# wisamreid/HcUnet

Measured on AMD Instinct MI355X. Metric: training voxels/sec (fwd+bwd+step), 5-level 3D U-Net, 256×256×16×4 tiles, higher is better.
Workload: dtype fp32; 1 GPU; config 2: 3D U-Net feature_sizes=[8,16,32,64,128] fp32 train step (fwd + pixel BCE + bwd + Adam), B=2 per GPU, 256x256x16x4 volumes; global_batch=2, per_gpu_batch=2, input_dtype=fp32, parallelism=dp1

## Files before the change

### hcunet_amd/csrc/common.h

```cpp
#pragma once
#include <hip/hip_runtime.h>
#include <hip/hip_ext.h>
#include <cstddef>
#include <cstdint>
#include <algorithm>
#include <cstdlib>
#include <string>

typedef float floatx4 __attribute__((ext_vector_type(4)));
typedef short shortx8 __attribute__((ext_vector_type(8)));
typedef short shortx4 __attribute__((ext_vector_type(4)));
typedef short shortx2 __attribute__((ext_vector_type(2)));
typedef float floatx2 __attribute__((ext_vector_type(2)));
typedef unsigned int u32x2 __attribute__((ext_vector_type(2)));
typedef unsigned int u32x4 __attribute__((ext_vector_type(4)));
typedef __bf16 bf16x2 __attribute__((ext_vector_type(2)));

namespace hcu {

struct ChainRec {
  hipStream_t s = nullptr;
  hipEvent_t ev = nullptr;
  unsigned long n = 0;
};
// ... 311 lines not shown
  f.Cout = Cout;
  f.Cin_g = Cin_g;
  f.groups = groups;
  f.fold_mod = fold_mod;
  f.part_c = part_c;
  f.part_cs = part_cs;
  f.ACs = ACs;
  return f;
}
inline PwWgArgs pw_wgrad_args(const WGradFinalize &f, const void *A, const void *G, long nvox,
                              int ACs, int GCs) {
  PwWgArgs g{};
  g.A = static_cast<const uint16_t *>(A);
  g.G = static_cast<const uint16_t *>(G);
  g.partial = const_cast<float *>(f.partial);
  g.nvox = nvox;
  g.per_block = (nvox + f.KB - 1) / f.KB;
  g.ACs = ACs;
  g.GCs = GCs;
  g.ACR = f.ACs;
  g.GCR = f.Ntot;
  g.Mtot = f.Mtot;
  g.Ntot = f.Ntot;
  g.bias_row = f.Mtot > f.T * f.ACs ? 1 : 0;
  return g;
}
int launch_wgrad_finalize(const WGradFinalize &f, hipStream_t s);
constexpr int kWgfBatch = 24;
int launch_wgrad_finalize_batch(const WGradFinalize *fs, int n, hipStream_t s);


int launch_bn_fwd_finalize(const float *stats, int R, int statsW, int C, int Cs,
                           double count, const float *gamma, const float *beta,
                           float *run_mean, float *run_var, int64_t *nbt,
                           float eps, float momentum, int training, BNCoef coef,
                           hipStream_t s);
int launch_bn_bwd_finalize(const float *part, int R, int C, int Cs, int W, double count,
                           BNCoef coef, float *dgamma, float *dbeta, int training,
                           int accumulate, hipStream_t s);

int launch_maxpool_fwd(const float *y, const float *scale, const float *shift,
                       float *p, int B, int X, int Y, int Z, int Cs,
                       int kx, int ky, int kz, hipStream_t s, int bf = 0);

int bwd_rows(int64_t nvox, int Cs);
int launch_bn_bwd_reduce_dense(float *dA, const float *y, BNCoef coef,
                               int64_t nvox, int Cs, float *part, int R,
                               hipStream_t s, int bf = 0);
int pool_bwd_rows(int B, int X, int Y, int Z, int Cs, int kx, int ky, int kz);
int launch_bn_bwd_reduce_pool(const float *dP, const float *y, BNCoef coef,
                              float *dz, int B, int X, int Y, int Z, int Cs,
                              int kx, int ky, int kz, float *part, int R,
                              hipStream_t s, int bf = 0);
int launch_bn_bwd_apply(float *dz, const float *y, BNCoef coef, int64_t nvox,
                        int Cs, hipStream_t s, int bf = 0);

int launch_outconv_fwd(const float *y, BNCoef coef, const float *w,
                       const float *bias, float *pred, int B, int64_t V, int C,
                       int Cs, int Co, hipStream_t s, int bf = 0);
int outconv_bwd_rows(int64_t nvox, int Cs);
int launch_outconv_bwd(const float *dpred, const float *y, BNCoef coef,
                       const float *w, float *dz, int B, int64_t V, int C,
                       int Cs, int Co, float *part_bn, float *part_oc, int R,
                       hipStream_t s, int bf = 0);

int chansum_rows(int64_t nvox, int Cs);
int launch_chansum(const float *x, int64_t nvox, int Cs, float *part, int R,
                   hipStream_t s, int bf = 0);
int launch_reduce_partials(const float *part, int R, int W, int n, float *out,
                           int accumulate, hipStream_t s);

int launch_to_cl(const float *x, float *xcl, int B, int C, int Cs, int64_t V,
                 hipStream_t s, int bf = 0, int x_dtype = 0);
int launch_from_cl(const float *xcl, float *x, int B, int C, int Cs, int64_t V,
                   hipStream_t s, int bf = 0);

struct WPack {
  int on, CK, S, ICs, CoutW;
};
inline WPack wpack_of(const GConvArgs &a) {
  WPack p{};
  if (a.use_bconv && a.bes == 4) {
    const int T = a.KX * a.KY * a.KZ, TPS = 16 / a.CK;
    p.on = 1;
    p.CK = a.CK;
    p.S = (T + TPS - 1) / TPS;
    p.ICs = a.ICs;
    p.CoutW = a.CoutW;
    return p;
  }
  if (a.use_bconv) {
    const int T = a.KX * a.KY * a.KZ, TPS = 32 / a.CK;
    p.on = 3;
    p.CK = a.CK;
    p.S = (T + TPS - 1) / TPS;
    p.ICs = a.ICs;
    p.CoutW = a.CoutW;
    return p;
  }
  if (a.use_conv8) {
    p.on = 2;
    p.CK = a.ICs / 4;
    p.S = a.KX * a.KY * a.KZ;
    p.ICs = a.ICs;
    p.CoutW = 8;
    return p;
// ... 105 lines not shown
```

### hcunet_amd/csrc/pointwise.hip

```cpp
#include "common.h"
#include "timing.h"
#include <algorithm>

namespace hcu {

__device__ __forceinline__ float bnrelu(float y, float sc, float sh) {
  return fmaxf(fmaf(y, sc, sh), 0.f);
}
__device__ __forceinline__ float4 ld4(const float *p) {
  return *reinterpret_cast<const float4 *>(p);
}
__device__ __forceinline__ void st4(float *p, float4 v) {
  *reinterpret_cast<float4 *>(p) = v;
}
struct bf16_t {
  uint16_t v;
};
__device__ __forceinline__ float4 ld4(const bf16_t *p) {
  const uint2 u = *reinterpret_cast<const uint2 *>(p);
  return make_float4(bf_lo(u.x), bf_hi(u.x), bf_lo(u.y), bf_hi(u.y));
}
__device__ __forceinline__ void st4(bf16_t *p, float4 v) {
  *reinterpret_cast<uint2 *>(p) = make_uint2(pack_bf2(v.x, v.y), pack_bf2(v.z, v.w));
}
// ... 309 lines not shown
}

int launch_maxpool_fwd(const float *y, const float *scale, const float *shift,
                       float *p, int B, int X, int Y, int Z, int Cs, int kx, int ky,
                       int kz, hipStream_t s, int bf) {
  const int PX = X / kx, PY = Y / ky, PZ = Z / kz;
  const int64_t n = (int64_t)B * PX * PY * PZ * (Cs / 4);
  if (n >= (int64_t)1 << 31) return fail(4, "max_pool3d: more than 2^31 channel quads per launch");
  if (kx == 2 && ky == 2 && kz == 1 && n > 0) {
    const int N = bf ? 8 : 4;
    if (Cs % N == 0) {
      const int64_t nv = (int64_t)B * PX * PY * PZ * (Cs / N);
      HCU_TIMED(s, "maxpool221_kernel", 0.0, (double)(bf ? 2 : 4) * Cs * ((double)B * X * Y * Z + (double)B * PX * PY * PZ),
                HCU_BF_DISPATCH(bf, maxpool221_kernel, dim3((unsigned)((nv + 255) / 256)), dim3(256), 0, s,
                                (const T *)y, scale, shift, (T *)p, X, Y, Z, Cs, PX, PY, (uint32_t)nv,
                                pool_div(Cs * 4 / N, PX, PY, PZ)));
      HCU_CHECK_LAUNCH();
      return 0;
    }
  }
  HCU_TIMED(s, "maxpool_fwd_kernel", 0.0, 0.0,
            HCU_BF_DISPATCH(bf, maxpool_fwd_kernel, dim3(grid_for(n)), dim3(256), 0, s,
                            (const T *)y, scale, shift, (T *)p, B, X, Y, Z, Cs, kx, ky, kz, PX,
                            PY, PZ, pool_div(Cs, PX, PY, PZ)));
  HCU_CHECK_LAUNCH();
  return 0;
}

struct RedGeom {
  int tb;
  int64_t chunk;
  int64_t total;
};
__host__ __device__ inline RedGeom red_geom(int64_t nvox, int Cs, int R) {
  RedGeom g;
  const int C4 = Cs / 4;
  g.tb = C4 <= 256 ? (256 / C4) * C4 : C4;
  g.total = nvox * C4;
  int64_t per = (g.total + R - 1) / R;
  g.chunk = (per + g.tb - 1) / g.tb * g.tb;
  return g;
}
int bwd_rows(int64_t nvox, int Cs) {
  const int C4 = Cs / 4;
  const int tb = C4 <= 256 ? (256 / C4) * C4 : C4;
  const int64_t total = nvox * C4;
  int64_t r = (total + (int64_t)tb * 4 - 1) / ((int64_t)tb * 4);
  return (int)std::max<int64_t>(1, std::min<int64_t>(r, 1024));
}
int chansum_rows(int64_t nvox, int Cs) { return bwd_rows(nvox, Cs); }
int outconv_bwd_rows(int64_t nvox, int Cs) { return bwd_rows(nvox, Cs); }

template <int NV>
__device__ void block_reduce_c4(float (&v)[NV], float *lds, int tb, int C4,
                                float *out_row ) {
  const int tid = threadIdx.x;
  if (tid < tb)
    for (int k = 0; k < NV; ++k) lds[tid * NV + k] = v[k];
  __syncthreads();
  if (tid < C4) {
    float acc[NV];
    for (int k = 0; k < NV; ++k) acc[k] = 0.f;
    for (int t = tid; t < tb; t += C4)
      for (int k = 0; k < NV; ++k) acc[k] += lds[t * NV + k];
    for (int k = 0; k < NV; ++k) out_row[tid * NV + k] = acc[k];
  }
}

template <typename T>
__global__ void __launch_bounds__(256)
bn_bwd_reduce_dense_kernel(T *dA, const T *y, BNCoef coef, int64_t nvox,
                           int Cs, float *part, RedGeom g) {
  extern __shared__ __attribute__((aligned(16))) float lds[];
  const int C4 = Cs / 4, tid = threadIdx.x;
  float v[8] = {0, 0, 0, 0, 0, 0, 0, 0};
  if (tid < g.tb) {
    const int64_t beg = (int64_t)blockIdx.x * g.chunk;
    const int64_t end = std::min(beg + g.chunk, g.total);
    const int c = (int)((beg + tid) % C4) * 4;
    const float4 sc = ld4(coef.scale + c), sh = ld4(coef.shift + c);
    const float4 mu = ld4(coef.mean + c), is = ld4(coef.invstd + c);
    for (int64_t e = beg + tid; e < end; e += g.tb) {
      const size_t off = (size_t)e * 4;
      const float4 yy = ld4(y + off);
      float4 d = ld4(dA + off);
      d.x = fmaf(yy.x, sc.x, sh.x) > 0.f ? d.x : 0.f;
      d.y = fmaf(yy.y, sc.y, sh.y) > 0.f ? d.y : 0.f;
      d.z = fmaf(yy.z, sc.z, sh.z) > 0.f ? d.z : 0.f;
      d.w = fmaf(yy.w, sc.w, sh.w) > 0.f ? d.w : 0.f;
      st4(dA + off, d);
      v[0] += d.x;
      v[1] = fmaf(d.x, (yy.x - mu.x) * is.x, v[1]);
      v[2] += d.y;
      v[3] = fmaf(d.y, (yy.y - mu.y) * is.y, v[3]);
      v[4] += d.z;
      v[5] = fmaf(d.z, (yy.z - mu.z) * is.z, v[5]);
      v[6] += d.w;
      v[7] = fmaf(d.w, (yy.w - mu.w) * is.w, v[7]);
    }
  }
  block_reduce_c4<8>(v, lds, g.tb, C4, part + (size_t)blockIdx.x * Cs * 2);
}

int launch_bn_bwd_reduce_dense(float *dA, const float *y, BNCoef coef, int64_t nvox,
                               int Cs, float *part, int R, hipStream_t s, int bf) {
  const RedGeom g = red_geom(nvox, Cs, R);
  HCU_TIMED(s, "bn_bwd_reduce_dense_kernel", 0.0, 2.0 * nvox * Cs * (bf ? 2 : 4),
            HCU_BF_DISPATCH(bf, bn_bwd_reduce_dense_kernel, dim3(R), dim3(256),
                            (size_t)std::max(g.tb, 256) * 8 * 4, s, (T *)dA, (const T *)y, coef,
                            nvox, Cs, part, g));
  HCU_CHECK_LAUNCH();
  return 0;
}

template <typename T>
__global__ void __launch_bounds__(256)
bn_bwd_reduce_pool_kernel(const T *dP, const T *y, BNCoef coef, T *dz,
                          int B, int X, int Y, int Z, int Cs, int kx, int ky, int kz,
                          float *part, RedGeom g, PoolDiv dv) {
// ... 19 lines not shown
      float4 m = make_float4(-INFINITY, -INFINITY, -INFINITY, -INFINITY);
      int4 am = make_int4(-1, -1, -1, -1);
      int idx = 0;
      for (int i = 0; i < kx; ++i)
        for (int j = 0; j < ky; ++j)
          for (int k = 0; k < kz; ++k, ++idx) {
            const float4 t = ld4(y + ((((size_t)b * X + x0 + i) * Y + y0 + j) * Z + z0 + k) * Cs + c);
            const float a0 = bnrelu(t.x, sc.x, sh.x), a1 = bnrelu(t.y, sc.y, sh.y);
            const float a2 = bnrelu(t.z, sc.z, sh.z), a3 = bnrelu(t.w, sc.w, sh.w);
            if (a0 > m.x) { m.x = a0; am.x = idx; }
            if (a1 > m.y) { m.y = a1; am.y = idx; }
            if (a2 > m.z) { m.z = a2; am.z = idx; }
            if (a3 > m.w) { m.w = a3; am.w = idx; }
          }
      const float4 gp = ld4(dP + ((((size_t)b * PX + wx) * PY + wy) * PZ + wz) * Cs + c);
      for (int x = x0; x < x1; ++x)
        for (int yy = y0; yy < y1; ++yy)
          for (int z = z0; z < z1; ++z) {
            const size_t off = ((((size_t)b * X + x) * Y + yy) * Z + z) * Cs + c;
            float4 d = make_float4(0.f, 0.f, 0.f, 0.f);
            const bool inwin = x < x0 + kx && yy < y0 + ky && z < z0 + kz;
            if (inwin) {
              const int own = ((x - x0) * ky + (yy - y0)) * kz + (z - z0);
              const float4 yv = ld4(y + off);
              const float4 zv = make_float4(fmaf(yv.x, sc.x, sh.x), fmaf(yv.y, sc.y, sh.y),
                                            fmaf(yv.z, sc.z, sh.z), fmaf(yv.w, sc.w, sh.w));
              d.x = (am.x == own && zv.x > 0.f) ? gp.x : 0.f;
              d.y = (am.y == own && zv.y > 0.f) ? gp.y : 0.f;
              d.z = (am.z == own && zv.z > 0.f) ? gp.z : 0.f;
              d.w = (am.w == own && zv.w > 0.f) ? gp.w : 0.f;
              v[0] += d.x;
              v[1] = fmaf(d.x, (yv.x - mu.x) * is.x, v[1]);
              v[2] += d.y;
              v[3] = fmaf(d.y, (yv.y - mu.y) * is.y, v[3]);
              v[4] += d.z;
              v[5] = fmaf(d.z, (yv.z - mu.z) * is.z, v[5]);
              v[6] += d.w;
              v[7] = fmaf(d.w, (yv.w - mu.w) * is.w, v[7]);
            }
            st4(dz + off, d);
          }
    }
  }
  block_reduce_c4<8>(v, lds, g.tb, C4, part + (size_t)blockIdx.x * Cs * 2);
}

template <int N>
struct Win221 {
  float a[4][N], gp[N];
  int wx, wy, wz, b;
  bool ok;
};
template <typename T>
__global__ void __launch_bounds__(256)
bn_bwd_reduce_pool221_kernel(const T *dP, const T *y, BNCoef coef, T *dz, int X, int Y, int Z,
                             int Cs, float *part, RedGeom g, PoolDiv dv) {
  constexpr int N = VN<T>::N;
  extern __shared__ __attribute__((aligned(16))) float lds[];
  const int G = Cs / N, tid = threadIdx.x;
  const int PX = X / 2, PY = Y / 2;
  const size_t sy = (size_t)Z * Cs, sx = (size_t)Y * sy;
  float v[2 * N];
#pragma unroll
  for (int k = 0; k < 2 * N; ++k) v[k] = 0.f;
  if (tid < g.tb) {
    const int64_t beg = (int64_t)blockIdx.x * g.chunk;
    const int64_t end = std::min(beg + g.chunk, g.total);
    const int c = (int)((beg + tid) % G) * N;
    float sc[N], sh[N], mu[N], is[N];
    ldc<N>(coef.scale + c, sc);
    ldc<N>(coef.shift + c, sh);
    ldc<N>(coef.mean + c, mu);
    ldc<N>(coef.invstd + c, is);
    auto load = [&](int64_t e, Win221<N> &w) {
      w.ok = e < end;
      if (!w.ok) return;
      int q, gg;
      dv.c4.divmod((uint32_t)e, q, gg);
      dv.pz.divmod((uint32_t)q, q, w.wz);
      dv.py.divmod((uint32_t)q, q, w.wy);
      dv.px.divmod((uint32_t)q, w.b, w.wx);
      const size_t base = (((size_t)w.b * X + 2 * w.wx) * Y + 2 * w.wy) * sy + (size_t)w.wz * Cs + c;
      ldv(y + base, w.a[0]);
      ldv(y + base + sy, w.a[1]);
      ldv(y + base + sx, w.a[2]);
      ldv(y + base + sx + sy, w.a[3]);
      ldv(dP + ((((size_t)w.b * PX + w.wx) * PY + w.wy) * Z + w.wz) * Cs + c, w.gp);
    };
    auto finish = [&](const Win221<N> &w) {
      if (!w.ok) return;
      float d[4][N];
#pragma unroll
      for (int j = 0; j < N; ++j) {
        float m = -INFINITY;
        int am = -1;
        float zz[4];
#pragma unroll
        for (int t = 0; t < 4; ++t) {
          zz[t] = fmaf(w.a[t][j], sc[j], sh[j]);
          const float q = fmaxf(zz[t], 0.f);
          if (q > m) { m = q; am = t; }
        }
#pragma unroll
        for (int t = 0; t < 4; ++t) d[t][j] = (am == t && zz[t] > 0.f) ? w.gp[j] : 0.f;
      }
      const size_t base = (((size_t)w.b * X + 2 * w.wx) * Y + 2 * w.wy) * sy + (size_t)w.wz * Cs + c;
      stv(dz + base, d[0]);
      stv(dz + base + sy, d[1]);
      stv(dz + base + sx, d[2]);
      stv(dz + base + sx + sy, d[3]);
#pragma unroll
      for (int t = 0; t < 4; ++t)
#pragma unroll
        for (int j = 0; j < N; ++j) {
          v[2 * j] += d[t][j];
          v[2 * j + 1] = fmaf(d[t][j], (w.a[t][j] - mu[j]) * is[j], v[2 * j + 1]);
        }
      const bool lx = w.wx == PX - 1 && X > 2 * PX, ly = w.wy == PY - 1 && Y > 2 * PY;
      if (lx || ly) {
        float zero[N];
#pragma unroll
        for (int j = 0; j < N; ++j) zero[j] = 0.f;
        const int x1 = lx ? X : 2 * w.wx + 2, y1 = ly ? Y : 2 * w.wy + 2;
        for (int x = 2 * w.wx; x < x1; ++x)
          for (int yy = 2 * w.wy; yy < y1; ++yy)
            if (x >= 2 * w.wx + 2 || yy >= 2 * w.wy + 2)
              stv(dz + (((size_t)w.b * X + x) * Y + yy) * sy + (size_t)w.wz * Cs + c, zero);
      }
    };
    for (int64_t e = beg + tid; e < end; e += 2 * (int64_t)g.tb) {
      Win221<N> w0, w1;
      load(e, w0);
      load(e + g.tb, w1);
      finish(w0);
      finish(w1);
    }
  }
  if (tid < g.tb)
#pragma unroll
    for (int k = 0; k < 2 * N; ++k) lds[tid * 2 * N + k] = v[k];
  __syncthreads();
  if (tid < G) {
    float acc[2 * N];
#pragma unroll
    for (int k = 0; k < 2 * N; ++k) acc[k] = 0.f;
    for (int t = tid; t < g.tb; t += G)
#pragma unroll
      for (int k = 0; k < 2 * N; ++k) acc[k] += lds[t * 2 * N + k];
    float *out = part + (size_t)blockIdx.x * Cs * 2 + (size_t)tid * 2 * N;
#pragma unroll
    for (int k = 0; k < 2 * N; ++k) out[k] = acc[k];
  }
}

int pool_bwd_rows(int B, int X, int Y, int Z, int Cs, int kx, int ky, int kz) {
  return bwd_rows((int64_t)B * (X / kx) * (Y / ky) * (Z / kz), Cs);
}

int launch_bn_bwd_reduce_pool(const float *dP, const float *y, BNCoef coef, float *dz,
                              int B, int X, int Y, int Z, int Cs, int kx, int ky,
                              int kz, float *part, int R, hipStream_t s, int bf) {
  const RedGeom g = red_geom((int64_t)B * (X / kx) * (Y / ky) * (Z / kz), Cs, R);
  if (g.total >= (int64_t)1 << 31) return fail(4, "max_pool3d backward: more than 2^31 channel quads");
  const int N = bf ? 8 : 4;
  if (kx == 2 && ky == 2 && kz == 1 && Cs % N == 0) {
    const RedGeom gv = red_geom((int64_t)B * (X / 2) * (Y / 2) * Z, Cs * 4 / N, R);
    HCU_TIMED(s, "bn_bwd_reduce_pool221_kernel", 0.0,
              (double)(bf ? 2 : 4) * Cs * ((double)B * (X / 2) * (Y / 2) * Z + 2.0 * B * X * Y * Z),
              HCU_BF_DISPATCH(bf, bn_bwd_reduce_pool221_kernel, dim3(R), dim3(256),
                              (size_t)std::max(gv.tb, 256) * 2 * N * 4, s, (const T *)dP, (const T *)y,
                              coef, (T *)dz, X, Y, Z, Cs, part, gv, pool_div(Cs * 4 / N, X / 2, Y / 2, Z)));
    HCU_CHECK_LAUNCH();
    return 0;
  }
  HCU_TIMED(s, "bn_bwd_reduce_pool_kernel", 0.0, 0.0,
            HCU_BF_DISPATCH(bf, bn_bwd_reduce_pool_kernel, dim3(R), dim3(256),
                            (size_t)std::max(g.tb, 256) * 8 * 4, s, (const T *)dP, (const T *)y,
                            coef, (T *)dz, B, X, Y, Z, Cs, kx, ky, kz, part, g,
                            pool_div(Cs, X / kx, Y / ky, Z / kz)));
  HCU_CHECK_LAUNCH();
  return 0;
}

template <typename T>
__global__ void __launch_bounds__(256)
bn_bwd_apply_kernel(T *dz, const T *y, BNCoef coef, int64_t n4, int C4) {
  const int64_t i0 = (int64_t)blockIdx.x * 256 + threadIdx.x;
  const int64_t st = (int64_t)gridDim.x * 256;
  const int c = (int)(i0 % C4) * 4;
  const float4 sc = ld4(coef.scale + c), c1 = ld4(coef.c1 + c), c0 = ld4(coef.c0 + c);
  auto f = [&](float4 d, float4 yy) {
    d.x = fmaf(d.x, sc.x, fmaf(c1.x, yy.x, c0.x));
    d.y = fmaf(d.y, sc.y, fmaf(c1.y, yy.y, c0.y));
    d.z = fmaf(d.z, sc.z, fmaf(c1.z, yy.z, c0.z));
    d.w = fmaf(d.w, sc.w, fmaf(c1.w, yy.w, c0.w));
    return d;
  };
  int64_t i = i0;
  for (; i + 3 * st < n4; i += 4 * st) {
    float4 yy[4], d[4];
#pragma unroll
    for (int u = 0; u < 4; ++u) {
      yy[u] = ld4(y + (i + u * st) * 4);
      d[u] = ld4(dz + (i + u * st) * 4);
    }
#pragma unroll
    for (int u = 0; u < 4; ++u) st4(dz + (i + u * st) * 4, f(d[u], yy[u]));
  }
  for (; i < n4; i += st) st4(dz + i * 4, f(ld4(dz + i * 4), ld4(y + i * 4)));
}

template <typename T>
__global__ void __launch_bounds__(256)
bn_bwd_apply_vec_kernel(T *dz, const T *y, BNCoef coef, int64_t nv, int G) {
  constexpr int N = VN<T>::N;
  const int64_t i0 = (int64_t)blockIdx.x * 256 + threadIdx.x;
  const int64_t st = (int64_t)gridDim.x * 256;
  const int c = (int)(i0 % G) * N;
// ... 98 lines not shown
                            s, (const T *)y, coef, w, bias, pred, B, V, C, Cs, Co));
  HCU_CHECK_LAUNCH();
  return 0;
}

template <typename T>
__global__ void __launch_bounds__(256)
outconv_bwd_kernel(const float *dpred, const T *y, BNCoef coef, const float *w,
                   T *dz, int B, int64_t V, int C, int Cs, int Co, float *part_bn,
                   float *part_oc, RedGeom g) {
  extern __shared__ __attribute__((aligned(16))) float lds[];
  constexpr int NV = 8 + 5 * MAXCO;
  const int C4 = Cs / 4, tid = threadIdx.x;
  float v[NV];
  for (int k = 0; k < NV; ++k) v[k] = 0.f;
  if (tid < g.tb) {
    const int64_t beg = (int64_t)blockIdx.x * g.chunk;
    const int64_t end = std::min(beg + g.chunk, g.total);
    const int c = (int)((beg + tid) % C4) * 4;
    const float4 sc = ld4(coef.scale + c), sh = ld4(coef.shift + c);
    const float4 mu = ld4(coef.mean + c), is = ld4(coef.invstd + c);
    float wv[MAXCO][4];
    for (int o = 0; o < MAXCO; ++o)
      for (int j = 0; j < 4; ++j) wv[o][j] = (o < Co && c + j < C) ? w[o * C + c + j] : 0.f;
    for (int64_t e = beg + tid; e < end; e += g.tb) {
      const int64_t vox = e / C4;
      const int b = (int)(vox / V);
      const int64_t vv = vox % V;
      const size_t off = (size_t)vox * Cs + c;
      const float4 yy = ld4(y + off);
      float dp[MAXCO];
      for (int o = 0; o < MAXCO; ++o) dp[o] = o < Co ? dpred[((size_t)b * Co + o) * V + vv] : 0.f;
      const float yv[4] = {yy.x, yy.y, yy.z, yy.w};
      const float scv[4] = {sc.x, sc.y, sc.z, sc.w}, shv[4] = {sh.x, sh.y, sh.z, sh.w};
      const float muv[4] = {mu.x, mu.y, mu.z, mu.w}, isv[4] = {is.x, is.y, is.z, is.w};
      float dzv[4];
      for (int j = 0; j < 4; ++j) {
        const float z = fmaf(yv[j], scv[j], shv[j]);
        const float a = fmaxf(z, 0.f);
        float dA = 0.f;
        for (int o = 0; o < MAXCO; ++o) {
          dA = fmaf(dp[o], wv[o][j], dA);
          v[8 + o * 4 + j] = fmaf(dp[o], a, v[8 + o * 4 + j]);
        }
        dzv[j] = z > 0.f ? dA : 0.f;
        v[2 * j] += dzv[j];
        v[2 * j + 1] = fmaf(dzv[j], (yv[j] - muv[j]) * isv[j], v[2 * j + 1]);
      }
      if (c == 0)
        for (int o = 0; o < MAXCO; ++o) v[8 + 4 * MAXCO + o] += dp[o];
      st4(dz + off, make_float4(dzv[0], dzv[1], dzv[2], dzv[3]));
    }
  }
  if (tid < g.tb)
    for (int k = 0; k < NV; ++k) lds[tid * NV + k] = v[k];
  __syncthreads();
  if (tid < C4) {
    float acc[NV];
    for (int k = 0; k < NV; ++k) acc[k] = 0.f;
    for (int t = tid; t < g.tb; t += C4)
      for (int k = 0; k < NV; ++k) acc[k] += lds[t * NV + k];
    const int c = tid * 4;
    float *pb = part_bn + (size_t)blockIdx.x * Cs * 2;
    for (int k = 0; k < 8; ++k) pb[c * 2 + k] = acc[k];
    float *po = part_oc + (size_t)blockIdx.x * (Co * Cs + Co);
    for (int o = 0; o < Co; ++o)
      for (int j = 0; j < 4; ++j) po[o * Cs + c + j] = acc[8 + o * 4 + j];
    if (tid == 0)
      for (int o = 0; o < Co; ++o) po[Co * Cs + o] = acc[8 + 4 * MAXCO + o];
  }
}

int launch_outconv_bwd(const float *dpred, const float *y, BNCoef coef, const float *w,
                       float *dz, int B, int64_t V, int C, int Cs, int Co, float *part_bn,
                       float *part_oc, int R, hipStream_t s, int bf) {
  if (Co > MAXCO) return fail(4, "out_conv: out_channels > 4 not supported");
  const RedGeom g = red_geom((int64_t)B * V, Cs, R);
  const size_t lds = (size_t)std::max(g.tb, 256) * (8 + 5 * MAXCO) * 4;
  HCU_TIMED(s, "outconv_bwd_kernel", 0.0, 0.0,
            HCU_BF_DISPATCH(bf, outconv_bwd_kernel, dim3(R), dim3(256), lds, s, dpred,
                            (const T *)y, coef, w, (T *)dz, B, V, C, Cs, Co, part_bn, part_oc,
                            g));
  HCU_CHECK_LAUNCH();
  return 0;
}

template <typename T>
__global__ void __launch_bounds__(256)
chansum_kernel(const T *x, int Cs, float *part, RedGeom g) {
  extern __shared__ __attribute__((aligned(16))) float lds[];
  const int C4 = Cs / 4, tid = threadIdx.x;
  float v[4] = {0, 0, 0, 0};
  if (tid < g.tb) {
    const int64_t beg = (int64_t)blockIdx.x * g.chunk;
    const int64_t end = std::min(beg + g.chunk, g.total);
    for (int64_t e = beg + tid; e < end; e += g.tb) {
      const float4 t = ld4(x + e * 4);
      v[0] += t.x;
      v[1] += t.y;
      v[2] += t.z;
      v[3] += t.w;
    }
  }
  block_reduce_c4<4>(v, lds, g.tb, C4, part + (size_t)blockIdx.x * Cs);
}

int launch_chansum(const float *x, int64_t nvox, int Cs, float *part, int R, hipStream_t s,
                   int bf) {
  const RedGeom g = red_geom(nvox, Cs, R);
  HCU_TIMED(s, "chansum_kernel", 0.0, 0.0,
            HCU_BF_DISPATCH(bf, chansum_kernel, dim3(R), dim3(256),
                            (size_t)std::max(g.tb, 256) * 4 * 4, s, (const T *)x, Cs, part, g));
  HCU_CHECK_LAUNCH();
  return 0;
}

__device__ __forceinline__ double block_sum_column(const float *part, int R, int W, int j) {
  __shared__ double red[256];
  const int tid = threadIdx.x;
  double s = 0.0;
  for (int r = tid; r < R; r += 256) s += (double)part[(size_t)r * W + j];
  red[tid] = s;
// ... 189 lines not shown
```

### hcunet_amd/csrc/unet.cpp

```cpp
#include "common.h"
#include "timing.h"
#include "../../include/hcunet.h"
#include <algorithm>
#include <cstdio>
#include <cstdlib>
#include <cstring>
#include <initializer_list>
#include <mutex>
#include <string>
#include <vector>

namespace hcu {
static thread_local std::string g_err;
void set_error(const std::string &msg) { g_err = msg; }
int fail(int code, const std::string &msg) {
  g_err = msg;
  return code;
}
int launch_outconv_wfinalize(const float *part_oc, int R, int Co, int C, int Cs, float *dw,
                             float *db, int accumulate, hipStream_t s);
int launch_bn_count_increment(int64_t *const *ptrs, int n, hipStream_t s);
}

using namespace hcu;
// ... 1024 lines not shown
                         c.kpart(), c.s))
      return e;
  return 0;
}

PwArgs pw_args(const ConvLayer &L, bool dgrad, const float *in, const float *w, const float *bias, float *out) {
  PwArgs a{};
  a.in = reinterpret_cast<const uint16_t *>(in);
  a.w = w;
  a.bias = dgrad ? nullptr : bias;
  a.out = reinterpret_cast<uint16_t *>(out);
  a.nvox = L.out.vox();
  a.ICs = dgrad ? L.out.Cs : L.in.Cs;
  a.OCs = dgrad ? L.in.Cs : L.out.Cs;
  a.Cin = L.Cin_g;
  a.Cout = L.Cout;
  a.part_c = L.part_c;
  a.part_cs = L.part_cs;
  a.dgrad = dgrad ? 1 : 0;
  return a;
}

int conv_forward(const Ctx &c, const ConvLayer &L, const float *in, const float *isc,
                 const float *ish, int training, int in_fmt = 0, float *xcl_out = nullptr) {
  HCU_HIP(hipGetLastError());
  tag(L.name, "fwd");
  GConvArgs a = bind_conv(L.fwd, in, isc, ish, in_fmt ? c.P + L.w_off : c.image(L.wf_off), c.param(L.b_off),
                          c.fptr(c.sv, L.y_off), training ? c.part() : nullptr, c.kpart());
  a.in_fmt = in_fmt;
  a.in_c = in_fmt ? L.in.C : 0;
  a.xcl = xcl_out;
  const BNCoef coef = coef_at(c.sv, L.bn);
  if (int e = launch_conv_any(a, c.s)) return e;
  return launch_bn_fwd_finalize(c.part(), gconv_rows(L.fwd), L.fwd.CoutW, L.bn.C, L.bn.Cs,
                                L.bn.count, c.P + L.bn.gamma, c.P + L.bn.beta,
                                c.t.bn_running_mean[L.bn.index], c.t.bn_running_var[L.bn.index],
                                c.t.bn_num_batches_tracked[L.bn.index], c.p.spec.bn_eps,
                                c.p.spec.bn_momentum, training, coef, c.s);
}

bool fuse_bnbwd(Ctx &c, GConvArgs &a, const ConvLayer *bnl) {
  static const bool off = getenv("HCU_NO_BNFUSE") != nullptr;
  if (off || !bnl || !conv_bnbwd_fusable(a)) return false;
  const BNCoef coef = coef_at(c.sv, bnl->bn);
  a.bn_y = c.fptr(c.sv, bnl->y_off);
  a.bn_scale = coef.scale;
  a.bn_shift = coef.shift;
  a.bn_mean = coef.mean;
  a.bn_invstd = coef.invstd;
  a.stats = c.part();
  return true;
}

int finish_bn(const Ctx &c, const ConvLayer &bnl, int R, int W, float *dz, int training, int accumulate) {
  const BNCoef coef = coef_at(c.sv, bnl.bn);
  if (int e = launch_bn_bwd_finalize(c.part(), R, bnl.bn.C, bnl.bn.Cs, W, bnl.bn.count, coef,
                                     c.G + bnl.bn.gamma, c.G + bnl.bn.beta, training, accumulate, c.s))
    return e;
  return launch_bn_bwd_apply(dz, c.fptr(c.sv, bnl.y_off), coef, bnl.out.vox(), bnl.out.Cs, c.s, c.bf());
}

int finish_bnbwd(const Ctx &c, const GConvArgs &a, const ConvLayer &bnl, float *dz, int training,
                 int accumulate) {
  return finish_bn(c, bnl, gconv_rows(a), a.CoutW, dz, training, accumulate);
}

int convt_dgrad(Ctx &c, const ConvTLayer &u, const float *dU, float *dP, const ConvLayer *bnl, int training,
                int accumulate, bool &fused) {
  GConvArgs a = bind_conv(u.dgrad, dU, nullptr, nullptr, c.image(u.wd_off), nullptr, dP, nullptr, c.kpart());
  fused = fuse_bnbwd(c, a, bnl);
  if (int e = launch_conv_any(a, c.s)) return e;
  if (!fused) return 0;
  tag(bnl->name, "bnbwd");
  return finish_bnbwd(c, a, *bnl, dP, training, accumulate);
}

int conv_backward(Ctx &c, const ConvLayer &L, const float *A, const float *asc,
                  const float *ash, const float *dy, int dy_slot, float *dA, int accumulate,
                  const ConvLayer *bnl = nullptr, int training = 1, bool *bn_done = nullptr,
                  float *colsum = nullptr, bool wg_late = false);

int run_wgrad(Ctx &c, const WGradJob &j, const float *A, const float *a_scale, const float *a_shift,
              const float *G, float *dw, float *db, int accumulate) {
  WGradFinalize f = j.f;
  float *slab = nullptr;
  if (j.pw_blocks && !a_scale) {
    if (int e = c.slab(j.pw_slab, slab)) return e;
    f.partial = slab;
    f.KB = j.pw_blocks;
    const PwWgArgs pa = pw_wgrad_args(f, A, G, wgrad_gvox(j.w), j.w.ACs, j.w.GCs);
    if (int e = launch_pw_wgrad(pa, j.pw_blocks, c.wstream())) return e;
  } else {
    if (int e = c.slab(j.slab, slab)) return e;
    WGradArgs w = j.w;
    w.A = A;
    w.a_scale = a_scale;
    w.a_shift = a_shift;
    w.G = G;
    w.partial = slab;
    if (int e = launch_wgrad(w, c.wstream())) return e;
    f.partial = slab;
  }
  f.dw = dw;
  f.db = db;
  f.accumulate = accumulate;
  return c.pend_wgf(f);
}

WGradFinalize wgf_colsum(int mode, const float *rows, int R, int W, int Cout, float *db, int accumulate) {
  WGradFinalize f{};
  f.partial = rows;
  f.db = db;
  f.KB = R;
  f.Mtot = 1;
  f.Ntot = W;
  f.mode = mode;
  f.Cout = Cout;
  f.accumulate = accumulate;
  return f;
}

int conv_wgrad(Ctx &c, const ConvLayer &L, const float *A, const float *asc, const float *ash,
               const float *dy, int dy_slot, int accumulate) {
  tag(L.name, "wgrad");
  if (int e = c.fork()) return e;
  if (int e = run_wgrad(c, L.wg, A, asc, ash, dy, c.G + L.w_off, c.grad(L.b_off), accumulate))
    return e;
  return c.read_done(dy_slot);
}

int conv_backward(Ctx &c, const ConvLayer &L, const float *A, const float *asc,
                  const float *ash, const float *dy, int dy_slot, float *dA, int accumulate,
                  const ConvLayer *bnl, int training, bool *bn_done, float *colsum, bool wg_late) {
  if (!wg_late || !dA)
    if (int e = conv_wgrad(c, L, A, asc, ash, dy, dy_slot, accumulate)) return e;
  if (!dA) return 0;
  tag(L.name, "dgrad");
  if (L.pw && !bnl && !colsum) {
    if (int e = launch_pw(pw_args(L, true, dy, c.P + L.w_off, nullptr, dA), c.s)) return e;
    return wg_late ? conv_wgrad(c, L, A, asc, ash, dy, dy_slot, accumulate) : 0;
  }
  GConvArgs a = bind_conv(L.dgrad, dy, nullptr, nullptr, c.image(L.wd_off), nullptr, dA, colsum, c.kpart());
  const bool fused = fuse_bnbwd(c, a, bnl);
  if (int e = launch_conv_any(a, c.s)) return e;
  if (wg_late)
    if (int e = conv_wgrad(c, L, A, asc, ash, dy, dy_slot, accumulate)) return e;
  if (!fused) return 0;
  tag(bnl->name, "bnbwd");
  if (int e = finish_bnbwd(c, a, *bnl, dA, training, accumulate)) return e;
  if (bn_done) *bn_done = true;
  return 0;
}

int bn_backward(const Ctx &c, const ConvLayer &L, float *dbuf, const float *pool_dP,
                const int *pool_k, int training, int accumulate) {
  tag(L.name, "bnbwd");
  const BNCoef coef = coef_at(c.sv, L.bn);
  const float *y = c.fptr(c.sv, L.y_off);
  const int64_t nvox = L.out.vox();
  const int R = bwd_rows(nvox, L.out.Cs);
  if (pool_dP) {
    if (int e = launch_bn_bwd_reduce_pool(pool_dP, y, coef, dbuf, L.out.B, L.out.X, L.out.Y,
                                          L.out.Z, L.out.Cs, pool_k[0], pool_k[1], pool_k[2],
                                          c.part(), R, c.s, c.bf()))
      return e;
  } else {
    if (int e = launch_bn_bwd_reduce_dense(dbuf, y, coef, nvox, L.out.Cs, c.part(), R, c.s,
                                           c.bf()))
      return e;
  }
  return finish_bn(c, L, R, L.bn.Cs, dbuf, training, accumulate);
}

}

namespace {

int graphs_forced() {
  static const int v = [] {
    const char *e = getenv("HCU_GRAPHS");
    return e ? (e[0] == '1' ? 1 : 0) : -1;
  }();
  return v;
}
bool graphs_for(const hcu_unet_plan &p, bool backward) {
  const int f = graphs_forced();
  if (f >= 0) return f == 1;
  return !backward && p.fwd_flops < 100e9;
}

void append_bn_key(std::vector<uintptr_t> &key, const hcu_unet_plan &p, const hcu_unet_tensors *t) {
  for (int i = 0; i < p.n_bn; ++i) {
    key.push_back(t->bn_running_mean ? (uintptr_t)t->bn_running_mean[i] : 0);
    key.push_back(t->bn_running_var ? (uintptr_t)t->bn_running_var[i] : 0);
    key.push_back(t->bn_num_batches_tracked ? (uintptr_t)t->bn_num_batches_tracked[i] : 0);
  }
}

template <class F>
int run_graphed(const hcu_unet_plan &p, std::vector<uintptr_t> key, hipStream_t s, F enqueue) {
  if (!graphs_for(p, key[0] != 0) || timing_on()) return enqueue(s);
  int dev = 0;
  HCU_HIP(hipGetDevice(&dev));
  key.push_back((uintptr_t)dev);
  std::lock_guard<std::mutex> lk(p.gmu);
  for (auto &g : p.graphs)
    if (g.key == key) {
      g.used = ++p.gclock;
      HCU_HIP(hipGraphLaunch(g.exec, s));
      return HCU_OK;
    }
  if (!p.cap_stream || p.cap_device != dev) {
    if (p.cap_stream) (void)hipStreamDestroy(p.cap_stream);
// ... 1086 lines not shown
```

Baseline: 1.098 billion voxels/s.

## Split pooled BN backward into stats pass and fused pool-grad apply pass

For 2x2x1 maxpool followed by BN backward, the old path wrote the pooled-routing gradient dz, reduced stats, then ran a separate BN apply that re-read dz and y. The new path first runs a stats-only kernel that recomputes the routing without writing dz, finalizes the BN coefficients, then runs an apply kernel that recomputes the routing from dP and y and writes the final dz directly. This removes one full write and read of dz at the cost of reading y twice. Block reductions are also reworked so all 256 threads cooperate in the LDS sum with an unrolled loop, where before only C4 threads did it.

```diff
diff --git a/hcunet_amd/csrc/common.h b/hcunet_amd/csrc/common.h
--- a/hcunet_amd/csrc/common.h
+++ b/hcunet_amd/csrc/common.h
@@ -387,6 +387,13 @@
                               float *dz, int B, int X, int Y, int Z, int Cs,
                               int kx, int ky, int kz, float *part, int R,
                               hipStream_t s, int bf = 0);
+bool bn_bwd_pool221_vec(int Cs, int kx, int ky, int kz, int bf);
+int launch_bn_bwd_stats_pool221(const float *dP, const float *y, BNCoef coef, int B,
+                                int X, int Y, int Z, int Cs, float *part, int R,
+                                hipStream_t s, int bf = 0);
+int launch_bn_bwd_apply_pool221(const float *dP, const float *y, BNCoef coef,
+                                float *dz, int B, int X, int Y, int Z, int Cs,
+                                hipStream_t s, int bf = 0);
 int launch_bn_bwd_apply(float *dz, const float *y, BNCoef coef, int64_t nvox,
                         int Cs, hipStream_t s, int bf = 0);
 
diff --git a/hcunet_amd/csrc/pointwise.hip b/hcunet_amd/csrc/pointwise.hip
--- a/hcunet_amd/csrc/pointwise.hip
+++ b/hcunet_amd/csrc/pointwise.hip
@@ -385,19 +385,32 @@
 int outconv_bwd_rows(int64_t nvox, int Cs) { return bwd_rows(nvox, Cs); }
 
 template <int NV>
+__device__ __forceinline__ float group_sum(const float *lds, int tb, int C4, int c4, int k) {
+  float acc = 0.f;
+  int t = c4;
+  for (; t + 7 * C4 < tb; t += 8 * C4) {
+    float x[8];
+#pragma unroll
+    for (int u = 0; u < 8; ++u) x[u] = lds[(t + u * C4) * NV + k];
+#pragma unroll
+    for (int u = 0; u < 8; ++u) acc += x[u];
+  }
+  for (; t < tb; t += C4) acc += lds[t * NV + k];
+  return acc;
+}
+template <int NV>
+__device__ __forceinline__ void stage_sums(const float (&v)[NV], float *lds, int tb) {
+  const int tid = threadIdx.x;
+  if (tid < tb)
+#pragma unroll
+    for (int k = 0; k < NV; ++k) lds[tid * NV + k] = v[k];
+  __syncthreads();
+}
+template <int NV>
 __device__ void block_reduce_c4(float (&v)[NV], float *lds, int tb, int C4,
                                 float *out_row ) {
-  const int tid = threadIdx.x;
-  if (tid < tb)
-    for (int k = 0; k < NV; ++k) lds[tid * NV + k] = v[k];
-  __syncthreads();
-  if (tid < C4) {
-    float acc[NV];
-    for (int k = 0; k < NV; ++k) acc[k] = 0.f;
-    for (int t = tid; t < tb; t += C4)
-      for (int k = 0; k < NV; ++k) acc[k] += lds[t * NV + k];
-    for (int k = 0; k < NV; ++k) out_row[tid * NV + k] = acc[k];
-  }
+  stage_sums<NV>(v, lds, tb);
+  for (int i = threadIdx.x; i < C4 * NV; i += 256) out_row[i] = group_sum<NV>(lds, tb, C4, i / NV, i % NV);
 }
 
 template <typename T>
@@ -523,14 +536,67 @@
   bool ok;
 };
 template <typename T>
-__global__ void __launch_bounds__(256)
-bn_bwd_reduce_pool221_kernel(const T *dP, const T *y, BNCoef coef, T *dz, int X, int Y, int Z,
-                             int Cs, float *part, RedGeom g, PoolDiv dv) {
+struct Pool221 {
+  static constexpr int N = VN<T>::N;
+  const T *dP, *y;
+  int X, Y, Z, Cs, PX, PY, c;
+  size_t sy, sx;
+  PoolDiv dv;
+  __device__ Pool221(const T *dP_, const T *y_, int X_, int Y_, int Z_, int Cs_, int c_, const PoolDiv &dv_)
+      : dP(dP_), y(y_), X(X_), Y(Y_), Z(Z_), Cs(Cs_), PX(X_ / 2), PY(Y_ / 2), c(c_),
+        sy((size_t)Z_ * Cs_), sx((size_t)Y_ * Z_ * Cs_), dv(dv_) {}
+  __device__ __forceinline__ size_t base(const Win221<N> &w) const {
+    return (((size_t)w.b * X + 2 * w.wx) * Y + 2 * w.wy) * sy + (size_t)w.wz * Cs + c;
+  }
+  __device__ __forceinline__ void load(int64_t e, int64_t end, Win221<N> &w) const {
+    w.ok = e < end;
+    if (!w.ok) return;
+    int q, gg;
+    dv.c4.divmod((uint32_t)e, q, gg);
+    dv.pz.divmod((uint32_t)q, q, w.wz);
+    dv.py.divmod((uint32_t)q, q, w.wy);
+    dv.px.divmod((uint32_t)q, w.b, w.wx);
+    const size_t b0 = base(w);
+    ldv(y + b0, w.a[0]);
+    ldv(y + b0 + sy, w.a[1]);
+    ldv(y + b0 + sx, w.a[2]);
+    ldv(y + b0 + sx + sy, w.a[3]);
+    ldv(dP + ((((size_t)w.b * PX + w.wx) * PY + w.wy) * Z + w.wz) * Cs + c, w.gp);
+  }
+  __device__ __forceinline__ void grad(const Win221<N> &w, const float (&sc)[N], const float (&sh)[N],
+                                       float (&d)[4][N]) const {
+#pragma unroll
+    for (int j = 0; j < N; ++j) {
+      float m = -INFINITY;
+      int am = -1;
+      float zz[4];
+#pragma unroll
+      for (int t = 0; t < 4; ++t) {
+        zz[t] = fmaf(w.a[t][j], sc[j], sh[j]);
+        const float q = fmaxf(zz[t], 0.f);
+        if (q > m) { m = q; am = t; }
+      }
+#pragma unroll
+      for (int t = 0; t < 4; ++t) d[t][j] = (am == t && zz[t] > 0.f) ? w.gp[j] : 0.f;
+    }
+  }
+  template <class F>
+  __device__ __forceinline__ void dropped(const Win221<N> &w, F f) const {
+    const bool lx = w.wx == PX - 1 && X > 2 * PX, ly = w.wy == PY - 1 && Y > 2 * PY;
+    if (!(lx || ly)) return;
+    const int x1 = lx ? X : 2 * w.wx + 2, y1 = ly ? Y : 2 * w.wy + 2;
+    for (int x = 2 * w.wx; x < x1; ++x)
+      for (int yy = 2 * w.wy; yy < y1; ++yy)
+        if (x >= 2 * w.wx + 2 || yy >= 2 * w.wy + 2)
+          f((((size_t)w.b * X + x) * Y + yy) * sy + (size_t)w.wz * Cs + c);
+  }
+};
+template <typename T, bool WRITE_D>
+__device__ __forceinline__ void bn_bwd_reduce_pool221(const T *dP, const T *y, const BNCoef &coef, T *dz,
+                                                      int X, int Y, int Z, int Cs, float *part,
+                                                      const RedGeom &g, const PoolDiv &dv, float *lds) {
   constexpr int N = VN<T>::N;
-  extern __shared__ __attribute__((aligned(16))) float lds[];
   const int G = Cs / N, tid = threadIdx.x;
-  const int PX = X / 2, PY = Y / 2;
-  const size_t sy = (size_t)Z * Cs, sx = (size_t)Y * sy;
   float v[2 * N];
 #pragma unroll
   for (int k = 0; k < 2 * N; ++k) v[k] = 0.f;
@@ -543,43 +609,18 @@
     ldc<N>(coef.shift + c, sh);
     ldc<N>(coef.mean + c, mu);
     ldc<N>(coef.invstd + c, is);
-    auto load = [&](int64_t e, Win221<N> &w) {
-      w.ok = e < end;
-      if (!w.ok) return;
-      int q, gg;
-      dv.c4.divmod((uint32_t)e, q, gg);
-      dv.pz.divmod((uint32_t)q, q, w.wz);
-      dv.py.divmod((uint32_t)q, q, w.wy);
-      dv.px.divmod((uint32_t)q, w.b, w.wx);
-      const size_t base = (((size_t)w.b * X + 2 * w.wx) * Y + 2 * w.wy) * sy + (size_t)w.wz * Cs + c;
-      ldv(y + base, w.a[0]);
-      ldv(y + base + sy, w.a[1]);
-      ldv(y + base + sx, w.a[2]);
-      ldv(y + base + sx + sy, w.a[3]);
-      ldv(dP + ((((size_t)w.b * PX + w.wx) * PY + w.wy) * Z + w.wz) * Cs + c, w.gp);
-    };
+    const Pool221<T> p(dP, y, X, Y, Z, Cs, c, dv);
     auto finish = [&](const Win221<N> &w) {
       if (!w.ok) return;
       float d[4][N];
-#pragma unroll
-      for (int j = 0; j < N; ++j) {
-        float m = -INFINITY;
-        int am = -1;
-        float zz[4];
-#pragma unroll
-        for (int t = 0; t < 4; ++t) {
-          zz[t] = fmaf(w.a[t][j], sc[j], sh[j]);
-          const float q = fmaxf(zz[t], 0.f);
-          if (q > m) { m = q; am = t; }
-        }
-#pragma unroll
-        for (int t = 0; t < 4; ++t) d[t][j] = (am == t && zz[t] > 0.f) ? w.gp[j] : 0.f;
+      p.grad(w, sc, sh, d);
+      if (WRITE_D) {
+        const size_t base = p.base(w);
+        stv(dz + base, d[0]);
+        stv(dz + base + p.sy, d[1]);
+        stv(dz + base + p.sx, d[2]);
+        stv(dz + base + p.sx + p.sy, d[3]);
       }
-      const size_t base = (((size_t)w.b * X + 2 * w.wx) * Y + 2 * w.wy) * sy + (size_t)w.wz * Cs + c;
-      stv(dz + base, d[0]);
-      stv(dz + base + sy, d[1]);
-      stv(dz + base + sx, d[2]);
-      stv(dz + base + sx + sy, d[3]);
 #pragma unroll
       for (int t = 0; t < 4; ++t)
 #pragma unroll
@@ -587,45 +628,128 @@
           v[2 * j] += d[t][j];
           v[2 * j + 1] = fmaf(d[t][j], (w.a[t][j] - mu[j]) * is[j], v[2 * j + 1]);
         }
-      const bool lx = w.wx == PX - 1 && X > 2 * PX, ly = w.wy == PY - 1 && Y > 2 * PY;
-      if (lx || ly) {
-        float zero[N];
-#pragma unroll
-        for (int j = 0; j < N; ++j) zero[j] = 0.f;
-        const int x1 = lx ? X : 2 * w.wx + 2, y1 = ly ? Y : 2 * w.wy + 2;
-        for (int x = 2 * w.wx; x < x1; ++x)
-          for (int yy = 2 * w.wy; yy < y1; ++yy)
-            if (x >= 2 * w.wx + 2 || yy >= 2 * w.wy + 2)
-              stv(dz + (((size_t)w.b * X + x) * Y + yy) * sy + (size_t)w.wz * Cs + c, zero);
-      }
+      if (WRITE_D)
+        p.dropped(w, [&](size_t off) {
+          float zero[N];
+#pragma unroll
+          for (int j = 0; j < N; ++j) zero[j] = 0.f;
+          stv(dz + off, zero);
+        });
     };
     for (int64_t e = beg + tid; e < end; e += 2 * (int64_t)g.tb) {
       Win221<N> w0, w1;
-      load(e, w0);
-      load(e + g.tb, w1);
+      p.load(e, end, w0);
+      p.load(e + g.tb, end, w1);
       finish(w0);
       finish(w1);
     }
   }
-  if (tid < g.tb)
-#pragma unroll
-    for (int k = 0; k < 2 * N; ++k) lds[tid * 2 * N + k] = v[k];
-  __syncthreads();
-  if (tid < G) {
-    float acc[2 * N];
-#pragma unroll
-    for (int k = 0; k < 2 * N; ++k) acc[k] = 0.f;
-    for (int t = tid; t < g.tb; t += G)
-#pragma unroll
-      for (int k = 0; k < 2 * N; ++k) acc[k] += lds[t * 2 * N + k];
-    float *out = part + (size_t)blockIdx.x * Cs * 2 + (size_t)tid * 2 * N;
-#pragma unroll
-    for (int k = 0; k < 2 * N; ++k) out[k] = acc[k];
+  block_reduce_c4<2 * N>(v, lds, g.tb, G, part + (size_t)blockIdx.x * Cs * 2);
+}
+template <typename T>
+__global__ void __launch_bounds__(256)
+bn_bwd_reduce_pool221_kernel(const T *dP, const T *y, BNCoef coef, T *dz, int X, int Y, int Z,
+                             int Cs, float *part, RedGeom g, PoolDiv dv) {
+  extern __shared__ __attribute__((aligned(16))) float lds[];
+  bn_bwd_reduce_pool221<T, true>(dP, y, coef, dz, X, Y, Z, Cs, part, g, dv, lds);
+}
+template <typename T>
+__global__ void __launch_bounds__(256)
+bn_bwd_stats_pool221_kernel(const T *dP, const T *y, BNCoef coef, int X, int Y, int Z, int Cs,
+                            float *part, RedGeom g, PoolDiv dv) {
+  extern __shared__ __attribute__((aligned(16))) float lds[];
+  bn_bwd_reduce_pool221<T, false>(dP, y, coef, nullptr, X, Y, Z, Cs, part, g, dv, lds);
+}
+
+template <typename T>
+__global__ void __launch_bounds__(256)
+bn_bwd_apply_pool221_kernel(const T *dP, const T *y, BNCoef coef, T *dz, int X, int Y, int Z,
+                            int Cs, int64_t nw, PoolDiv dv) {
+  constexpr int N = VN<T>::N;
+  const int64_t i0 = (int64_t)blockIdx.x * 256 + threadIdx.x;
+  const int64_t st = (int64_t)gridDim.x * 256;
+  const int c = (int)(i0 % (Cs / N)) * N;
+  float sc[N], sh[N], c1[N], c0[N];
+  ldc<N>(coef.scale + c, sc);
+  ldc<N>(coef.shift + c, sh);
+  ldc<N>(coef.c1 + c, c1);
+  ldc<N>(coef.c0 + c, c0);
+  const Pool221<T> p(dP, y, X, Y, Z, Cs, c, dv);
+  auto apply = [&](float (&d)[N], const float (&yy)[N]) {
+#pragma unroll
+    for (int j = 0; j < N; ++j) d[j] = fmaf(d[j], sc[j], fmaf(c1[j], yy[j], c0[j]));
+  };
+  auto finish = [&](const Win221<N> &w) {
+    if (!w.ok) return;
+    float d[4][N];
+    p.grad(w, sc, sh, d);
+#pragma unroll
+    for (int t = 0; t < 4; ++t) apply(d[t], w.a[t]);
+    const size_t base = p.base(w);
+    stv(dz + base, d[0]);
+    stv(dz + base + p.sy, d[1]);
+    stv(dz + base + p.sx, d[2]);
+    stv(dz + base + p.sx + p.sy, d[3]);
+    p.dropped(w, [&](size_t off) {
+      float yy[N], o[N];
+      ldv(y + off, yy);
+#pragma unroll
+      for (int j = 0; j < N; ++j) o[j] = 0.f;
+      apply(o, yy);
+      stv(dz + off, o);
+    });
+  };
+  for (int64_t e = i0; e < nw; e += 2 * st) {
+    Win221<N> w0, w1;
+    p.load(e, nw, w0);
+    p.load(e + st, nw, w1);
+    finish(w0);
+    finish(w1);
   }
 }
 
 int pool_bwd_rows(int B, int X, int Y, int Z, int Cs, int kx, int ky, int kz) {
   return bwd_rows((int64_t)B * (X / kx) * (Y / ky) * (Z / kz), Cs);
+}
+
+bool bn_bwd_pool221_vec(int Cs, int kx, int ky, int kz, int bf) {
+  return kx == 2 && ky == 2 && kz == 1 && Cs % (bf ? 8 : 4) == 0;
+}
+
+int launch_bn_bwd_stats_pool221(const float *dP, const float *y, BNCoef coef, int B, int X, int Y,
+                                int Z, int Cs, float *part, int R, hipStream_t s, int bf) {
+  const int N = bf ? 8 : 4;
+  const int64_t nwin = (int64_t)B * (X / 2) * (Y / 2) * Z;
+  if (nwin * (Cs / 4) >= (int64_t)1 << 31) return fail(4, "max_pool3d backward: more than 2^31 channel quads");
+  const RedGeom gv = red_geom(nwin, Cs * 4 / N, R);
+  HCU_TIMED(s, "bn_bwd_stats_pool221_kernel", 0.0,
+            (double)(bf ? 2 : 4) * Cs * ((double)nwin + (double)B * X * Y * Z),
+            HCU_BF_DISPATCH(bf, bn_bwd_stats_pool221_kernel, dim3(R), dim3(256),
+                            (size_t)std::max(gv.tb, 256) * 2 * N * 4, s, (const T *)dP, (const T *)y,
+                            coef, X, Y, Z, Cs, part, gv, pool_div(Cs * 4 / N, X / 2, Y / 2, Z)));
+  HCU_CHECK_LAUNCH();
+  return 0;
+}
+
+int launch_bn_bwd_apply_pool221(const float *dP, const float *y, BNCoef coef, float *dz, int B, int X,
+                                int Y, int Z, int Cs, hipStream_t s, int bf) {
+  const int N = bf ? 8 : 4, G = Cs / N;
+  const int64_t nwin = (int64_t)B * (X / 2) * (Y / 2) * Z, nw = nwin * G;
+  if (nwin * (Cs / 4) >= (int64_t)1 << 31) return fail(4, "max_pool3d backward: more than 2^31 channel quads");
+  int64_t want = (nw + 511) / 512;
+  if (want < 512) want = (nw + 255) / 256;
+  int grid = (int)std::max<int64_t>(1, std::min<int64_t>(want, 65536));
+  if (256 % G) {
+    const int per = G / std::__gcd(256, G);
+    grid = std::max(per, grid / per * per);
+  }
+  HCU_TIMED(s, "bn_bwd_apply_pool221_kernel", 0.0,
+            (double)(bf ? 2 : 4) * Cs * ((double)nwin + 2.0 * B * X * Y * Z),
+            HCU_BF_DISPATCH(bf, bn_bwd_apply_pool221_kernel, dim3(grid), dim3(256), 0, s, (const T *)dP,
+                            (const T *)y, coef, (T *)dz, X, Y, Z, Cs, nw,
+                            pool_div(Cs * 4 / N, X / 2, Y / 2, Z)));
+  HCU_CHECK_LAUNCH();
+  return 0;
 }
 
 int launch_bn_bwd_reduce_pool(const float *dP, const float *y, BNCoef coef, float *dz,
@@ -634,7 +758,7 @@
   const RedGeom g = red_geom((int64_t)B * (X / kx) * (Y / ky) * (Z / kz), Cs, R);
   if (g.total >= (int64_t)1 << 31) return fail(4, "max_pool3d backward: more than 2^31 channel quads");
   const int N = bf ? 8 : 4;
-  if (kx == 2 && ky == 2 && kz == 1 && Cs % N == 0) {
+  if (bn_bwd_pool221_vec(Cs, kx, ky, kz, bf)) {
     const RedGeom gv = red_geom((int64_t)B * (X / 2) * (Y / 2) * Z, Cs * 4 / N, R);
     HCU_TIMED(s, "bn_bwd_reduce_pool221_kernel", 0.0,
               (double)(bf ? 2 : 4) * Cs * ((double)B * (X / 2) * (Y / 2) * Z + 2.0 * B * X * Y * Z),
@@ -839,22 +963,19 @@
       st4(dz + off, make_float4(dzv[0], dzv[1], dzv[2], dzv[3]));
     }
   }
-  if (tid < g.tb)
-    for (int k = 0; k < NV; ++k) lds[tid * NV + k] = v[k];
-  __syncthreads();
-  if (tid < C4) {
-    float acc[NV];
-    for (int k = 0; k < NV; ++k) acc[k] = 0.f;
-    for (int t = tid; t < g.tb; t += C4)
-      for (int k = 0; k < NV; ++k) acc[k] += lds[t * NV + k];
-    const int c = tid * 4;
-    float *pb = part_bn + (size_t)blockIdx.x * Cs * 2;
-    for (int k = 0; k < 8; ++k) pb[c * 2 + k] = acc[k];
-    float *po = part_oc + (size_t)blockIdx.x * (Co * Cs + Co);
-    for (int o = 0; o < Co; ++o)
-      for (int j = 0; j < 4; ++j) po[o * Cs + c + j] = acc[8 + o * 4 + j];
-    if (tid == 0)
-      for (int o = 0; o < Co; ++o) po[Co * Cs + o] = acc[8 + 4 * MAXCO + o];
+  stage_sums<NV>(v, lds, g.tb);
+  float *pb = part_bn + (size_t)blockIdx.x * Cs * 2;
+  float *po = part_oc + (size_t)blockIdx.x * (Co * Cs + Co);
+  for (int i = tid; i < C4 * NV; i += 256) {
+    const int c4 = i / NV, k = i % NV;
+    if (k < 8) {
+      pb[c4 * 8 + k] = group_sum<NV>(lds, g.tb, C4, c4, k);
+    } else if (k < 8 + 4 * MAXCO) {
+      const int o = (k - 8) / 4, j = (k - 8) % 4;
+      if (o < Co) po[o * Cs + c4 * 4 + j] = group_sum<NV>(lds, g.tb, C4, c4, k);
+    } else if (c4 == 0 && k - (8 + 4 * MAXCO) < Co) {
+      po[Co * Cs + k - (8 + 4 * MAXCO)] = group_sum<NV>(lds, g.tb, C4, 0, k);
+    }
   }
 }
 
diff --git a/hcunet_amd/csrc/unet.cpp b/hcunet_amd/csrc/unet.cpp
--- a/hcunet_amd/csrc/unet.cpp
+++ b/hcunet_amd/csrc/unet.cpp
@@ -1100,12 +1100,15 @@
   return true;
 }
 
+int finalize_bn(const Ctx &c, const ConvLayer &bnl, int R, int W, int training, int accumulate) {
+  return launch_bn_bwd_finalize(c.part(), R, bnl.bn.C, bnl.bn.Cs, W, bnl.bn.count, coef_at(c.sv, bnl.bn),
+                                c.G + bnl.bn.gamma, c.G + bnl.bn.beta, training, accumulate, c.s);
+}
+
 int finish_bn(const Ctx &c, const ConvLayer &bnl, int R, int W, float *dz, int training, int accumulate) {
-  const BNCoef coef = coef_at(c.sv, bnl.bn);
-  if (int e = launch_bn_bwd_finalize(c.part(), R, bnl.bn.C, bnl.bn.Cs, W, bnl.bn.count, coef,
-                                     c.G + bnl.bn.gamma, c.G + bnl.bn.beta, training, accumulate, c.s))
-    return e;
-  return launch_bn_bwd_apply(dz, c.fptr(c.sv, bnl.y_off), coef, bnl.out.vox(), bnl.out.Cs, c.s, c.bf());
+  if (int e = finalize_bn(c, bnl, R, W, training, accumulate)) return e;
+  return launch_bn_bwd_apply(dz, c.fptr(c.sv, bnl.y_off), coef_at(c.sv, bnl.bn), bnl.out.vox(), bnl.out.Cs, c.s,
+                             c.bf());
 }
 
 int finish_bnbwd(const Ctx &c, const GConvArgs &a, const ConvLayer &bnl, float *dz, int training,
@@ -1207,6 +1210,15 @@
   const float *y = c.fptr(c.sv, L.y_off);
   const int64_t nvox = L.out.vox();
   const int R = bwd_rows(nvox, L.out.Cs);
+  static const bool pool_dz = !(getenv("HCU_POOL_DZ") && getenv("HCU_POOL_DZ")[0] == '0');
+  if (pool_dP && pool_dz && bn_bwd_pool221_vec(L.out.Cs, pool_k[0], pool_k[1], pool_k[2], c.bf())) {
+    if (int e = launch_bn_bwd_stats_pool221(pool_dP, y, coef, L.out.B, L.out.X, L.out.Y, L.out.Z, L.out.Cs,
+                                            c.part(), R, c.s, c.bf()))
+      return e;
+    if (int e = finalize_bn(c, L, R, L.bn.Cs, training, accumulate)) return e;
+    return launch_bn_bwd_apply_pool221(pool_dP, y, coef, dbuf, L.out.B, L.out.X, L.out.Y, L.out.Z, L.out.Cs,
+                                       c.s, c.bf());
+  }
   if (pool_dP) {
     if (int e = launch_bn_bwd_reduce_pool(pool_dP, y, coef, dbuf, L.out.B, L.out.X, L.out.Y,
                                           L.out.Z, L.out.Cs, pool_k[0], pool_k[1], pool_k[2],
```

After: 1.106 billion voxels/s (median of 6 runs). No clear change (+0.7%).
